# mrcdr/lambda-lanczos

Hardware: AMD Instinct MI355X
Metric: Lanczos iterations/sec + SpMV GB/s (fp64, n=10M nnz=150M) at 1/2/4/8 GPUs (higher is better)
Workload: dtype f64; 1 GPU; random symmetric CSR n=10000000 nnz=150000000 fp64; n=10000000, nnz=150000000, partition=single GPU, orth_mode=0, tridiag_mode=2, eps=engine default

## Files before the change

lambda-lanczos_amd/_capi.py:

```python
import ctypes as C
import os

_HERE = os.path.dirname(os.path.abspath(__file__))
LIB_PATH = os.environ.get("LL_LIB_PATH") or os.path.join(_HERE, "lib", "liblanczos_hip.so")
GEN_PATH = os.path.join(_HERE, "lib", "libllgen.so")
HEADER_PATH = os.path.join(os.path.dirname(_HERE), "include", "lanczos_hip.h")

LL_OK, LL_ERR_INVALID, LL_ERR_HIP, LL_ERR_RCCL, LL_ERR_ALLOC, LL_ERR_CALLBACK = range(6)
ORTH_CGS_DGKS, ORTH_CGS2, ORTH_MGS = 0, 1, 2
TRIDIAG_QR, TRIDIAG_BISECT, TRIDIAG_AUTO = 0, 1, 2
SPMV_CSR_STREAM, SPMV_PB, SPMV_TILED, SPMV_SYM = 0, 1, 2, 3
UPPER, LOWER = 0, 1
ACCURACY_DEFAULT, ACCURACY_NORMWISE, ACCURACY_COMPONENTWISE = 0, 1, 2
UNIQUE_ID_BYTES = 128
EXPO_MULTI_MAX = 16


ABI_VERSION = (0, 5)


class LanczosHipError(RuntimeError):
    def __init__(self, code, msg):
        super().__init__("liblanczos_hip error %d: %s" % (code, msg))
        self.code = code
# ... 65 lines not shown
        ("seconds_host_tridiag", f64),
        ("seconds_spmv", f64),
        ("seconds_orth", f64),
        ("last_alpha_len", i64),
        ("seconds_host_enqueue", f64),
        ("seconds_host_wait", f64),
        ("seconds_setup", f64),
        ("seconds_finish", f64),
        ("second_passes", i64),
        ("seconds_comm_gather", f64),
        ("seconds_comm_allreduce", f64),
        ("lagged_iterations", i64),
        ("pair_iterations", i64),
        ("pair_gate_trips", i64),
        ("workspace_vectors", i64),
        ("replay_mismatches", i64),
        ("reserved", i64 * 4),
    ]

    def as_dict(self):
        d = {k: getattr(self, k) for k, _ in self._fields_ if k != "reserved"}
        d["block_iterations"] = int(self.reserved[0])
        d["block_flushed_vectors"] = int(self.reserved[1])
        return d


P = C.POINTER
PROTOTYPES = {
    "ll_last_error": (C.c_char_p, []),
    "ll_version": (C.c_int, []),
    "ll_abi_check": (C.c_int, [C.c_int, C.c_int, C.c_size_t, C.c_size_t]),
    "ll_ctx_create": (C.c_int, [C.c_int, P(vp)]),
    "ll_ctx_create_on_stream": (C.c_int, [C.c_int, vp, P(vp)]),
    "ll_ctx_destroy": (C.c_int, [vp]),
    "ll_ctx_stream": (C.c_int, [vp, P(vp)]),
    "ll_ctx_synchronize": (C.c_int, [vp]),
    "ll_ctx_release_cache": (C.c_int, [vp]),
    "ll_ctx_reload_env": (C.c_int, [vp]),
    "ll_ctx_set_tuning": (C.c_int, [vp, C.c_char_p, C.c_char_p]),
    "ll_ctx_set_profiling": (C.c_int, [vp, C.c_int]),
    "ll_timer_start": (C.c_int, [vp]),
    "ll_timer_stop": (C.c_int, [vp, P(f64)]),
    "ll_bandwidth_probe": (C.c_int, [vp, C.c_size_t, P(f64), P(f64)]),
    "ll_comm_unique_id": (C.c_int, [vp]),
    "ll_comm_init": (C.c_int, [vp, vp, C.c_int, C.c_int]),
    "ll_comm_rank": (C.c_int, [vp, P(C.c_int), P(C.c_int)]),
# ... 136 lines not shown
```

lambda-lanczos_amd/csrc/context.cpp:

```cpp
#include <algorithm>
#include <cstdlib>
#include <memory>

#include "engine.hpp"

namespace ll {
static thread_local std::string g_last_error;
void set_error(const std::string& msg) { g_last_error = msg; }
}

using namespace ll;

namespace ll {
namespace {
long long to_ll(const std::string& v) { return std::atoll(v.c_str()); }
bool to_flag(const std::string& v) { return std::atoi(v.c_str()) != 0; }
int Tuning::*pauli_bits_key(const std::string& key) {
  static const std::pair<const char*, int Tuning::*> keys[] = {
      {"pauli_tile_bits", &Tuning::pauli_tile_bits}, {"pauli_sector_block_bits", &Tuning::pauli_sector_block_bits},
      {"pauli_momentum_block_bits", &Tuning::pauli_momentum_block_bits},
      {"pauli_momentum_full_block_bits", &Tuning::pauli_momentum_full_block_bits},
      {"pauli_symmetric_block_bits", &Tuning::pauli_symmetric_block_bits},
      {"pauli_block_expand_block_bits", &Tuning::pauli_block_expand_block_bits},
      {"pauli_block_project_block_bits", &Tuning::pauli_block_project_block_bits},
      {"pauli_rdm_tile_bits", &Tuning::pauli_rdm_tile_bits}, {"pauli_rdm_block_bits", &Tuning::pauli_rdm_block_bits}};
  for (const auto& k : keys)
    if (key == k.first) return k.second;
  return nullptr;
}
}
bool tuning_apply(Tuning& t, const std::string& key, const std::string& v) {
  const Tuning d;
  const bool e = v.empty();
  if (key == "spmv_kernel") t.spmv_kernel = v == "csr" ? LL_SPMV_CSR_STREAM : (v == "pb" ? LL_SPMV_PB : (v == "tiled" ? LL_SPMV_TILED : -1));
  else if (key == "spmv_keep_both") t.keep_both = e ? d.keep_both : to_flag(v);
  else if (key == "pb_phase2") t.pb_phase2 = v == "atomic" ? LL_PB_ATOMIC : (v == "ordered" ? LL_PB_ORDERED : LL_PB_FIXED);
  else if (key == "pb_placements") t.pb_placements = e ? d.pb_placements : (int)std::max<long long>(1, std::min<long long>(16, to_ll(v)));
  else if (key == "pb_placement_trace") t.pb_placement_trace = e ? false : to_flag(v);
  else if (key == "comm_overlap") t.comm_overlap = e ? d.comm_overlap : to_flag(v);
  else if (key == "gather_chunks") t.gather_chunks = e ? 0 : (int)std::max<long long>(0, to_ll(v));
  else if (key == "csr_split") t.csr_split = e ? d.csr_split : to_flag(v);
  else if (key == "iter_trace") t.iter_trace = v;
  else if (key == "sharded_norm") t.sharded_norm_measured = v == "measured";
  else if (key == "pair_gs") t.pair_gs = e ? d.pair_gs : to_flag(v);
  else if (key == "block_gs") t.block_gs = e ? d.block_gs : to_flag(v);
  else if (key == "pb_diag") t.pb_diag = e ? d.pb_diag : to_flag(v);
  else if (key == "fuse_launches") {
    const long long level = e ? 2 : to_ll(v);
    t.fuse_launches = level >= 1;
    t.lagged_gs = level >= 2;
  } else if (key == "blas_small_bytes") t.blas_small_bytes = e ? d.blas_small_bytes : to_ll(v);
  else if (key == "tridiag_thread") t.tridiag_thread = e ? d.tridiag_thread : to_flag(v);
  else if (key == "tridiag_lag") t.tridiag_lag = e ? d.tridiag_lag : (int)to_ll(v);
  else if (key == "dgks_threshold") t.dgks_threshold = e ? d.dgks_threshold : std::atof(v.c_str());
  else if (key == "slab_bytes") t.slab_bytes = e ? d.slab_bytes : std::max<long long>(1, to_ll(v));
  else if (key == "pb_block") t.pb_block = e ? 0 : (int)std::max<long long>(0, to_ll(v));
  else if (key == "pb_row_block") t.pb_row_block = e ? 0 : (int)std::max<long long>(0, to_ll(v));
  else if (key == "pb_col_block") t.pb_col_block = e ? 0 : (int)std::max<long long>(0, to_ll(v));
  else if (key == "pb_threads1") {
    t.pb_threads1 = e ? 0 : (int)to_ll(v);
    if (t.pb_threads1 != 256 && t.pb_threads1 != 512 && t.pb_threads1 != 1024) t.pb_threads1 = 0;
  } else if (key == "pb_pad") {
    t.pb_pad = e ? 0 : (int)to_ll(v);
    if (t.pb_pad != 4 && t.pb_pad != 16) t.pb_pad = 0;
  } else if (key == "pb_xpre") t.pb_xpre = e ? d.pb_xpre : to_flag(v);
  else if (key == "pb_test_all_remote") t.pb_test_all_remote = e ? false : to_flag(v);
  else if (key == "force_rp64") t.force_rp64 = e ? false : to_flag(v);
  else if (key == "spmv_tile_balance") t.spmv_tile_balance = e ? d.spmv_tile_balance : to_flag(v);
  else if (int Tuning::*bits = pauli_bits_key(key)) t.*bits = e ? d.*bits : (int)std::max<long long>(0, std::min<long long>(30, to_ll(v)));
// ... 476 lines not shown
```

lambda-lanczos_amd/csrc/engine.hpp:

```cpp
#pragma once

#include <chrono>
#include <complex>
#include <functional>
#include <map>
#include <system_error>
#include <thread>

#include "ll_internal.hpp"

namespace ll {

constexpr int kScalAlpha = 0, kScalNorms = 8, kScalScratch = 32, kScalSpare = 40, kScalZero = 63, kScalCount = 64;

inline double now_s() {
  return std::chrono::duration<double>(std::chrono::steady_clock::now().time_since_epoch()).count();
}
inline int64_t round_up(int64_t v, int64_t m) { return (v + m - 1) / m * m; }
inline bool is_device_ptr(const void* p) {
  if (p == nullptr) return false;
  hipPointerAttribute_t a;
  if (hipPointerGetAttributes(&a, p) != hipSuccess) {
    (void)hipGetLastError();
    return false;
  }
  return a.type == hipMemoryTypeDevice;
}
inline void host_copy(void* dst, const void* src, size_t bytes) {
  constexpr size_t kParallelFrom = (size_t)8 << 20;
  constexpr int kThreads = 4;
  if (bytes < kParallelFrom) {
    std::memcpy(dst, src, bytes);
    return;
  }
  const size_t piece = ((bytes / kThreads) + 4095) & ~(size_t)4095;
  std::thread th[kThreads - 1];
// ... 174 lines not shown
```

lambda-lanczos_amd/csrc/gs_block.hip:

```cpp
#include <algorithm>

#include "gs_strips.hpp"

namespace ll {

namespace {
__device__ __forceinline__ void block_sum2_all(double& a, double& b, double* sh) {
  a = wave_sum(a);
  b = wave_sum(b);
  const int lane = threadIdx.x & 63, wave = threadIdx.x >> 6;
  __syncthreads();
  if (lane == 0) {
    sh[wave] = a;
    sh[4 + wave] = b;
  }
  __syncthreads();
  a = (sh[0] + sh[1]) + (sh[2] + sh[3]);
  b = (sh[4] + sh[5]) + (sh[6] + sh[7]);
}
__device__ __forceinline__ void block_max2_all(double& a, double& b, double* sh) {
#pragma unroll
  for (int d = 32; d > 0; d >>= 1) {
    a = fmax(a, __shfl_down(a, d, 64));
    b = fmax(b, __shfl_down(b, d, 64));
// ... 69 lines not shown
    const double* prev = s == 1 ? dk : p + (size_t)(s - 2) * pstride;
    const double pinv = s == 1 ? 1.0 : 1.0 / sqrt(*sc.nsq[s - 2]);
    const double es = *sc.e[s];
    double* out = p + (size_t)s * pstride;
    for (int i = tid; i < RW; i += 256) {
      const double t = block_tri_row(hist_alpha, hist_beta, in, i, reals, W, alpha_k);
      out[i] = (t - es * in[i]) * inv - nin * (prev[i] * pinv);
    }
    __syncthreads();
  }
  for (int i = tid; i < RW; i += 256) {
    const double ir = 1.0 / sqrt(rho2[i / reals]);
    prA[i] = p[(size_t)(m - 1) * pstride + i] * ir;
    prB[i] = m >= 2 ? p[(size_t)(m - 2) * pstride + i] * ir : 0.0;
  }
}
void launch_block_predict(int k, int m, int reals, const BlockScalars& sc, const double* rho2, const double* cpk, double* hist_alpha,
                          const double* hist_beta, double* dk, double* p, int pstride, double* prA, double* prB, hipStream_t s) {
  hipLaunchKernelGGL(block_predict_kernel, dim3(1), dim3(256), 0, s, k, m, reals, sc, rho2, cpk, hist_alpha, hist_beta, dk, p, pstride, prA,
                     prB);
  LL_HIP(hipGetLastError());
}

template <typename T, int NV, int PC, int M>
__device__ __forceinline__ void block_trip_compute(const T (&ur)[NV][strip<T, PC>::EPT], int nv, const T (&b)[M][strip<T, PC>::EPT],
                                                   T (&cA)[strip<T, PC>::EPT], T (&cB)[strip<T, PC>::EPT],
                                                   const double* __restrict__ prAc, const double* __restrict__ prBc, double* mine,
                                                   int setstride, int lane) {
  constexpr int EPT = strip<T, PC>::EPT;
  double sre[M][NV], sim[M][NV];
#pragma unroll
  for (int v = 0; v < NV; ++v) {
    acc_t<T> ca, cb;
    const int vv = v < nv ? v : nv - 1;
    const bool real = v < nv;
    if constexpr (scalar_traits<T>::is_complex) {
      const double xa = ld_const(prAc, 2 * vv), ya = ld_const(prAc, 2 * vv + 1), xb = ld_const(prBc, 2 * vv), yb = ld_const(prBc, 2 * vv + 1);
      ca = zc{real ? xa : 0.0, real ? ya : 0.0};
      cb = zc{real ? xb : 0.0, real ? yb : 0.0};
    } else {
      const double xa = ld_const(prAc, vv), xb = ld_const(prBc, vv);
      ca = real ? xa : 0.0;
      cb = real ? xb : 0.0;
    }
    acc_t<T> sm[M];
#pragma unroll
    for (int i = 0; i < M; ++i) sm[i] = zero<acc_t<T>>();
#pragma unroll
    for (int e = 0; e < EPT; ++e) {
      fnma_acc(cA[e], ca, ur[v][e]);
      if constexpr (M >= 2) fnma_acc(cB[e], cb, ur[v][e]);
#pragma unroll
// ... 82 lines not shown
      load_lstrip_u<T, PC, FULL>(bv.part[0], base, n, cA);
      if constexpr (M >= 2) load_lstrip_u<T, PC, FULL>(bv.part[1], base, n, cB);
    }
    for (int t = 0; t < ntrips; t += 2) {
      __builtin_amdgcn_sched_barrier(0);
      issue(ub, t + 1);
      __builtin_amdgcn_sched_barrier(0);
      block_trip_compute<T, JB, PC, M>(ua, min(JB, Wl - JB * t), b, cA, cB, prAc + R * JB * t, prBc + R * JB * t, mine + R * JB * t, R * Wl, lane);
      if (t + 1 >= ntrips) break;
      __builtin_amdgcn_sched_barrier(0);
      issue(ua, t + 2);
      __builtin_amdgcn_sched_barrier(0);
      block_trip_compute<T, JB, PC, M>(ub, min(JB, Wl - JB * (t + 1)), b, cA, cB, prAc + R * JB * (t + 1), prBc + R * JB * (t + 1),
                                       mine + R * JB * (t + 1), R * Wl, lane);
    }
    store_lstrip_u<T, PC, FULL>(outA, base, n, cA);
    if constexpr (M >= 2) store_lstrip_u<T, PC, FULL>(outB, base, n, cB);
    if (!last) return;
#pragma unroll
    for (int e = 0; e < EPT; ++e) {
      b[M - 1][e] = cA[e];
      if constexpr (M >= 2) b[M - 2][e] = cB[e];
    }
    int at = 0;
#pragma unroll
    for (int i = 1; i < M; ++i) {
#pragma unroll
      for (int ip = 0; ip < i; ++ip) {
        acc_t<T> g = zero<acc_t<T>>();
#pragma unroll
        for (int e = 0; e < EPT; ++e) cfma_acc(g, b[ip][e], b[i][e]);
        const acc_t<T> gs = wave_sum(g);
        if (lane == 0) {
          if constexpr (scalar_traits<T>::is_complex) {
            tail[at] += gs.re;
            tail[at + 1] += gs.im;
          } else {
            tail[at] += gs;
          }
        }
        at += R;
      }
    }
#pragma unroll
    for (int i = 0; i < M; ++i) {
      double nn = 0.0;
// ... 13 lines not shown
  for (int i = tid; i < lcols; i += kBlock) {
    const double v = (lds[i] + lds[lcols + i]) + (lds[2 * lcols + i] + lds[3 * lcols + i]);
    int g;
    if (i < M * R * Wl) {
      const int set = i / (R * Wl);
      g = set * R * W + R * col0 + (i - set * R * Wl);
    } else {
      g = M * R * W + (i - M * R * Wl);
    }
    out[g] = v;
  }
}
constexpr int kBlockJB = 2;
template <typename T, int PC, int M>
static void block_sweep_launch(int grid, size_t lds_bytes, hipStream_t s, int64_t n, const T* const* vtab, int W, int col0, int Wl, int flags,
                               const BlockVecs<T>& bv, const double* prA, const double* prB, double* partials) {
  hipLaunchKernelGGL((block_sweep_kernel<T, PC, M, kBlockJB>), dim3(grid), dim3(kBlock), lds_bytes, s, n, vtab, W, col0, Wl, flags, bv, prA, prB,
                     partials);
}
template <typename T>
int launch_block_sweep(int64_t n, const T* const* vtab, int W, int m, const BlockVecs<T>& bv, const double* prA, const double* prB,
                       double* partials, int pieces, int per_launch, hipStream_t s) {
  constexpr int R = scalar_traits<T>::reals;
  LL_REQUIRE(m == 1 || m == 2 || m == 4, "internal: block sweep of 1, 2 or 4 iterations");
  const int64_t strips16k = (n * (int64_t)sizeof(T) + 16383) / 16384;
  int pc = strips16k >= kLaggedFullStrips ? 4 : 2;
  if (pieces == 2 || pieces == 4) pc = pieces;
  const int grid = pc == 4 ? strip_grid(n, strip<T, 4>::ELEMS) : strip_grid(n, strip<T, 2>::ELEMS);
  const int ng = R * m * (m - 1) / 2 + m;
  per_launch = std::max(1, std::min(per_launch, block_sweep_max_vecs<T>(m)));
  for (int col0 = 0; col0 < W; col0 += per_launch) {
    const int Wl = std::min(per_launch, W - col0);
    const int flags = (col0 == 0 ? kPairFirst : 0) | (col0 + Wl == W ? kPairLast : 0);
    const size_t lds_bytes = (size_t)4 * (size_t)(m * R * Wl + ((flags & kPairLast) ? ng : 0)) * sizeof(double);
#define LL_BLOCK_SWEEP(PC_, M_) block_sweep_launch<T, PC_, M_>(grid, lds_bytes, s, n, vtab, W, col0, Wl, flags, bv, prA, prB, partials)
    if (pc == 4) {
      if (m == 4) LL_BLOCK_SWEEP(4, 4);
      else if (m == 2) LL_BLOCK_SWEEP(4, 2);
      else LL_BLOCK_SWEEP(4, 1);
    } else {
      if (m == 4) LL_BLOCK_SWEEP(2, 4);
      else if (m == 2) LL_BLOCK_SWEEP(2, 2);
      else LL_BLOCK_SWEEP(2, 1);
    }
#undef LL_BLOCK_SWEEP
    LL_HIP(hipGetLastError());
  }
  return grid;
}

__global__ __launch_bounds__(256) void block_fold_kernel(const double* __restrict__ cols, int k, int m, int reals, BlockScalars sc,
                                                         const double* __restrict__ p, int pstride, double* __restrict__ rho2,
                                                         double* __restrict__ cpk, double* __restrict__ hist_alpha,
                                                         double* __restrict__ hist_beta, double* __restrict__ raw0,
                                                         double* __restrict__ raw1, BlockHost host) {
  __shared__ double red[8];
  const int tid = threadIdx.x;
  const int W = k + 1, RW = reals * W;
  const double* tail = cols + (size_t)m * RW;
  const double* diag = tail + reals * m * (m - 1) / 2;
  for (int s = 0; s < m; ++s) {
    const int j = k + 1 + s;
    double* raw = (s & 1) ? raw1 : raw0;
    const double* rawp = (s & 1) ? raw0 : raw1;
// ... 114 lines not shown
```

lambda-lanczos_amd/csrc/lanczos_loop.hpp:

```cpp
#pragma once

#include "engine.hpp"
#include "loop_support.hpp"
#include "raw_basis.hpp"
#include "ritz_tracker.hpp"
#include "trace.hpp"

#include <algorithm>
#include <cmath>
#include <limits>
#include <random>
#include <string>
#include <variant>

namespace ll {


template <typename T> struct LoopState {
  Engine<T>& E;
  Basis<T>& U;
  EventRing& ring;
  PhaseTimer& timer;
  int64_t nl;
  hipStream_t s;
// ... 44 lines not shown
  int64_t ld = 0;
  int64_t small_bytes = 0;

  int64_t max_k_hint = 0;
  bool pair_enabled = false;
  bool pair_allowed = true;
  int64_t n_pair = 0;
  int64_t n_gate_trips = 0;
  DevBuf<T> pwork[2];
  DevBuf<T> psplit;
  static constexpr size_t kPresizeCols = 4096;
  DevBuf<double> pbuf;
  static constexpr size_t kPairRec = (size_t)kLaggedMaxCols + 32;
  struct PairBuf {
    double* rec[4] = {nullptr, nullptr, nullptr, nullptr};
    double* zero = nullptr;
    double *p3 = nullptr, *p4 = nullptr;
    double* fold = nullptr;
    double* cols = nullptr;
    double* scal = nullptr;
    static constexpr size_t kDoubles = 10 * kPairRec + 64;
  } pb;
  bool slot_pair[kRingSlots] = {};
  int ev_of_slot[kRingSlots] = {0, 1, 2, 3, 4, 5, 6, 7};
  bool block_enabled = false;
  bool block_allowed = true;
  int64_t blk_k0 = 0;
  int64_t n_block = 0;
  int64_t n_block_flushed = 0;
  DevBuf<double> bbuf;
  DevBuf<T> bsplit[2];
  struct BlockBuf {
    double* rho2 = nullptr;
    double* cpk = nullptr;
    double* dk = nullptr;
    double* p = nullptr;
    double *prA = nullptr, *prB = nullptr;
    double *raw0 = nullptr, *raw1 = nullptr;
    double* cols = nullptr;
    double* nsq = nullptr;
    int64_t cap = 0;
    size_t rec = 0;
  } bb;
  static size_t block_row_at(int64_t j) { return ll::block_row_at(Engine<T>::R, j); }
  void enable_block() {
    constexpr size_t R = (size_t)Engine<T>::R;
    block_enabled = true;
    bb.cap = std::min<int64_t>(max_k_hint, (int64_t)kBlockMaxVecs) + 8;
    bb.rec = R * (size_t)(bb.cap + 8);
    const size_t tri = block_row_at(bb.cap) + R * (size_t)bb.cap;
    bbuf.alloc(E.ctx, (size_t)bb.cap + tri + 13 * bb.rec + 64);
    double* b = bbuf.p;
    bb.rho2 = carve(b, (size_t)bb.cap);
    bb.cpk = carve(b, tri);
    bb.dk = carve(b, bb.rec);
    bb.p = carve(b, 4 * bb.rec);
    bb.prA = carve(b, bb.rec);
    bb.prB = carve(b, bb.rec);
    bb.raw0 = carve(b, bb.rec);
    bb.raw1 = carve(b, bb.rec);
    bb.cols = carve(b, 4 * bb.rec + 32);
    bb.nsq = carve(b, 16);
  }
  static constexpr double kGate = sizeof(typename scalar_traits<T>::real) == 4 ? 2e-4 : kPairGate;
  DevBuf<const T*> vtab;
  static constexpr size_t kVtabCap = (size_t)kLaggedMaxCols + (size_t)kLaggedMaxLocked + 64;
  size_t vtab_chunks = 0;
  void vtab_begin_pass() {
    if (!vtab.p) return;
    launch_fill_ptrs<T>(vtab.p, 0, (int)std::min<int64_t>(n_locked, (int64_t)kVtabCap), locked, ld, s);
    vtab_chunks = 0;
  }
  const T* const* vtab_sync() {
    if (!vtab.p) return nullptr;
    for (; vtab_chunks < U.chunks.size(); ++vtab_chunks) {
      const int64_t start = n_locked + (int64_t)vtab_chunks * U.chunk_vecs;
      const int64_t count = std::min<int64_t>(U.chunk_vecs, (int64_t)kVtabCap - start);
      launch_fill_ptrs<T>(vtab.p, (int)start, (int)count, U.chunks[vtab_chunks], ld, s);
    }
    return vtab.p;
  }

  LoopState(Engine<T>& e, Basis<T>& u, EventRing& r, PhaseTimer& t, int64_t n_local, hipStream_t st)
      : E(e), U(u), ring(r), timer(t), nl(n_local), s(st) {}
  void configure(int64_t ld_, int64_t max_iteration, bool orth_dgks, bool defer_ok) {
// ... 45 lines not shown
      size_t p2 = kPresizeCols;
      while (p2 < cols) p2 *= 2;
      cols = p2;
    }
    E.ctx->ensure_partials((size_t)kMaxGrid * cols);
  }
  void bind_buffers() {
    E.ctx->ensure_h(LagBuf::kDoubles);
    double* b = E.ctx->h.get();
    for (auto& g : lb.g) g = carve(b, kHHalf);
    lb.hist_alpha = carve(b, kTOff);
    lb.hist_beta = carve(b, kTOff);
    lb.lambda = carve(b, (size_t)kLaggedMaxLocked);
  }
  void begin_pass(const NormRefs& refs0, const T* locked_vecs, int64_t n_lock, const double* lambda_shifted = nullptr,
                  double offset = 0.0, double norm_scale = 0.0) {
    refs_prev = refs0;
    pending = None{};
    locked = locked_vecs;
    n_locked = n_lock;
    pair_allowed = true;
    block_allowed = true;
    blk_k0 = 0;
    for (auto& b : slot_pair) b = false;
    lag_ok = lagged && n_lock <= kLaggedMaxLocked;
    lag_beta2_min = 0.0;
    if (lag_ok) vtab_begin_pass();
    if (lagged) {
      bind_buffers();
      constexpr size_t R = (size_t)Engine<T>::R;
      const size_t reach = (size_t)std::max<int64_t>(0, std::min<int64_t>(max_k_hint, (int64_t)kLaggedMaxCols)) + (size_t)n_lock + 2;
      const size_t cols = std::min<size_t>(kPresizeCols, (block_enabled ? 4 : 2) * R * reach + 6 * R + 4);
      E.ctx->ensure_partials((size_t)kMaxGrid * cols);
    }
    if (!lag_ok || n_lock == 0) return;
    const bool measure_theta = lambda_shifted == nullptr;
    if (!measure_theta) {
      LL_HIP(hipMemcpyAsync(lb.lambda, lambda_shifted, (size_t)n_lock * sizeof(double), hipMemcpyHostToDevice, s));
      LL_HIP(hipStreamSynchronize(s));
    }
    const BasisSegs<T> none = no_segs<T>(ld);
    E.ctx->ensure_partials(kMaxGrid);
    double* r2_dev = lb.g[0];
    for (int64_t i = 0; i < n_lock; ++i) {
      const T* z = locked + i * ld;
      T* y = work[0].p;
      E.apply(z, y, offset, measure_theta ? lb.lambda + i : nullptr, true);
      const ThreeTerm<T> tt{nullptr, z, lb.lambda + i, NormRefs{nullptr, nullptr, nullptr, 0}};
      const int grid = launch_mdot<T>(nl, y, none, tt, nullptr, E.ctx->partials.get(), small_bytes, s);
      launch_reduce_cols(E.ctx->partials.get(), grid, 1, r2_dev + i, nullptr, s);
    }
    E.all_reduce(r2_dev, (size_t)n_lock);
    std::vector<double> r2((size_t)n_lock), theta;
    E.fetch(r2_dev, r2.data(), (size_t)n_lock);
    if (measure_theta) {
// ... 158 lines not shown
    return basis;
  }
  int64_t enqueue_block(int64_t kk, double offset) {
    if constexpr (sizeof(typename scalar_traits<T>::real) == 8) return enqueue_block_f64(kk, offset);
    else return 0;
  }
  int64_t enqueue_block_f64(int64_t kk, double offset) {
    constexpr int R = Engine<T>::R;
    const Tuning& tune = E.ctx->tune;
    if (!block_enabled || !block_allowed || !pair_allowed || !lag_ok || n_locked != 0) return 0;
    const BlockIter* const bi = pending_as<BlockIter>();
    const LaggedIter* const lg = pending_as<LaggedIter>();
    int64_t k;
    if (bi) {
      if (bi->k + 1 != kk) return 0;
      k = bi->k;
    } else if (lg && lg->k == kk - 1 && kk >= 3) {
      k = kk - 1;
    } else {
      return 0;
    }
    const int64_t remaining = max_k_hint - (kk - 1);
    if (remaining < 1) return 0;
    const int m = remaining >= 4 ? 4 : (remaining >= 2 ? 2 : 1);
    const int64_t strips16k = (nl * (int64_t)sizeof(T) + 16383) / 16384;
    const bool streaming = tune.sweep_pipeline >= 2 || strips16k > 2 * kCUs + kCUs / 4;
    if (!streaming || vec_bytes() < stream_bytes() || k + m + 1 > bb.cap || (size_t)(k + m + 1) > kVtabCap) return 0;
    if (tune.pair_max_stored > 0 && k + 1 > tune.pair_max_stored) return 0;
    const int W = (int)(k + 1);
    const int ncols = m * R * W + R * m * (m - 1) / 2 + m;
    int per_launch = block_sweep_max_vecs<T>(m);
    if (tune.pair_split_vecs > 0) per_launch = std::min(per_launch, std::max(1, tune.pair_split_vecs));
    if (W > per_launch)
      for (auto& b : bsplit)
        if (!b.p) b.alloc(E.ctx, (size_t)ld);
    const double te0 = now_s();
    want_partial_cols((size_t)std::max(ncols, 1 + R));
    if (!bi) {
      LL_HIP(hipMemcpyAsync(U.vec(k), work[k & 1].p, (size_t)nl * sizeof(T), hipMemcpyDeviceToDevice, s));
      launch_block_enter((int)k, R, lb.g[k & 1], lg->c1, bb.rho2, bb.cpk, s);
      blk_k0 = k;
    }
    BlockVecs<T> bv{};
    for (int i = 0; i < m; ++i) bv.b[i] = U.vec(k + 1 + i);
    bv.part[0] = bsplit[0].p;
    bv.part[1] = bsplit[1].p;
    const T* const* vt = vtab_sync();
    BlockScalars sc{};
    BlockHost host{};
    int slots[4] = {0, 0, 0, 0};
    for (int i = 0; i < 4; ++i) {
      const int ii = std::min(i, m - 1);
      slots[i] = (int)((kk + ii) % kRingSlots);
      sc.e[i] = E.S(kScalAlpha + slots[i]);
      sc.nsq[i] = bb.nsq + 4 * ii;
      host.slot[i] = pinned_slot(slots[i]);
      host.gate[i] = pinned_gate(slots[i]);
    }
    for (int i = 0; i < m; ++i) {
      const T* x = i == 0 ? U.vec(k) : bv.b[i - 1];
      const T* xp = i == 0 ? U.vec(k - 1) : (i == 1 ? U.vec(k) : bv.b[i - 2]);
      const double* xn2 = i == 0 ? bb.rho2 + k : bb.nsq + 4 * (i - 1);
      const double* pn2 = i == 0 ? bb.rho2 + k - 1 : (i == 1 ? bb.rho2 + k : bb.nsq + 4 * (i - 2));
      double* e = E.S(kScalAlpha + slots[i]);
      timer.mark();
      typename Engine<T>::DeferredAlpha da;
      E.apply(x, bv.b[i], offset, e, true, fuse_launches ? &da : nullptr, nullptr, xn2);
      timer.mark();
      const int g3 = launch_pair_three_term<T>(nl, bv.b[i], x, xp, e, da.nparts > 0 ? da.partials : nullptr, da.nparts, xn2, pn2,
                                               E.ctx->partials.get(), false, s);
      launch_reduce_cols(E.ctx->partials.get(), g3, 1 + R, bb.nsq + 4 * i, nullptr, s);
      if (i + 1 < m) timer.mark();
    }
    launch_block_predict((int)k, m, R, sc, bb.rho2, bb.cpk, lb.hist_alpha, lb.hist_beta, bb.dk, bb.p, (int)bb.rec, bb.prA, bb.prB, s);
    const int grid = launch_block_sweep<T>(nl, vt, W, m, bv, bb.prA, bb.prB, E.ctx->partials.get(), tune.lagged_pieces, per_launch, s);
    launch_reduce_cols(E.ctx->partials.get(), grid, ncols, bb.cols, nullptr, s);
    const int ev = slots[m - 1];
    launch_block_fold(bb.cols, (int)k, m, R, sc, bb.p, (int)bb.rec, bb.rho2, bb.cpk, lb.hist_alpha, lb.hist_beta, bb.raw0, bb.raw1, host, s,
                      tune.event_in_launch ? ring.ev[ev] : nullptr);
    if (!tune.event_in_launch) LL_HIP(hipEventRecord(ring.ev[ev], s));
    timer.mark();
    for (int i = 0; i < m; ++i) {
      ev_of_slot[slots[i]] = ev;
      slot_pair[slots[i]] = true;
    }
    pending = BlockIter{k + m};
    n_block += m;
    if (m >= 2) n_pair += m;
    n_lagged += m;
    t_enqueue += now_s() - te0;
    return m;
  }
  bool enqueue_pair(int64_t k, double offset) {
    constexpr int R = Engine<T>::R;
    if (!pair_enabled || !pair_allowed || !lag_ok) return false;
    if (max_k_hint > 0 && k + 1 > max_k_hint) return false;
    const int64_t Lk = n_locked;
    PairIter in;
    if (const PairIter* pr = pending_as<PairIter>()) {
      if (pr->P + 2 != k) return false;
      in = *pr;
    } else if (const LaggedIter* lg = pending_as<LaggedIter>(); lg && lg->k == k - 1 && k >= 3) {
      in = PairIter{k - 2, {U.vec(k - 2), work[(k - 1) & 1].p}, {pb.zero, lb.g[(k - 1) & 1]}, {pb.scal + 0, lg->c1}, 0, 1};
    } else {
      return false;
    }
    const int64_t P = in.P;
    const T *const r1 = in.r[0], *const r2 = in.r[1];
    const double *const g1 = in.g[0], *const g2 = in.g[1], *const rho1sq = in.rho2[0], *const rho2sq = in.rho2[1];
    const int out_set = in.set ^ 1, out_rec = in.rec ^ 1;
// ... 200 lines not shown
    }
    RunList<T> runs;
    runs.ld = ld;
    if (full) runs = basis_runs(k);
    enqueue(k, offset, runs, mode);
    return 1;
  }
  void restart_after(int64_t j) {
    pending = None{};
    double* cj = E.S(kScalNorms + 3 * (int)(j % kRingSlots));
    refs_prev = NormRefs{cj, cj + 1, cj + 1, 0};
  }
  struct Scalars {
    double alpha, beta2, c0, c1;
    bool redone;
  };
  Scalars collect(int64_t j) {
    const int slot = (int)(j % kRingSlots);
    const double tw0 = now_s();
    LL_HIP(hipEventSynchronize(ring.ev[ev_of_slot[slot]]));
    t_wait += now_s() - tw0;
    const volatile double* hp = pinned_slot(slot);
    Scalars r{hp[0], hp[1], hp[2], hp[3], false};
    double* const beta2_dev = E.S(kScalNorms + 3 * slot) + 1;
    if (dgks && r.c1 < E.ctx->tune.dgks_threshold * r.c0) {
      if (r.c1 > 0.0 && std::isfinite(r.c1)) {
        const RunList<T> again = basis_runs(j);
        make_final(j);
        r.beta2 = r.c1 * E.second_pass(U.vec(j), again);
        ++n_second_passes;
        launch_set_scalar(beta2_dev, r.beta2, s);
        if (lag_ok) launch_set_scalar(lb.hist_beta + j - 1, std::sqrt(r.beta2), s);
        restart_after(j);
        r.redone = true;
      } else {
        r.beta2 = 0.0;
      }
    }
    if (!r.redone && lag_ok && n_locked > 0 && r.beta2 < lag_beta2_min) {
      make_final(j);
      lag_ok = false;
      restart_after(j);
      r.redone = true;
    }
    if (!r.redone && slot_pair[slot] && !(*pinned_gate(slot) <= kGate)) {
      pair_allowed = false;
// ... 86 lines not shown
  std::mt19937 mt(dev());
  std::uniform_real_distribution<Real> r((Real)-1, (Real)1);
  Real* f = reinterpret_cast<Real*>(v);
  for (int64_t i = 0; i < n * scalar_traits<T>::reals; ++i) f[i] = r(mt);
}

template <typename T>
void fill_stats(ll_run_stats* stats, LoopState<T>& loop, int64_t total_iterations, size_t last_alpha_len, double t_tridiag,
                double t_start) {
  ll_context* ctx = loop.E.ctx;
  if (stats) {
    std::memset(stats, 0, sizeof(*stats));
    stats->total_iterations = total_iterations;
    stats->seconds_host_tridiag = t_tridiag;
    stats->last_alpha_len = (int64_t)last_alpha_len;
    stats->seconds_host_enqueue = loop.t_enqueue;
    stats->seconds_host_wait = loop.t_wait;
    stats->second_passes = loop.n_second_passes;
    stats->lagged_iterations = loop.n_lagged;
    stats->pair_iterations = loop.n_pair;
    stats->pair_gate_trips = loop.n_gate_trips;
    stats->reserved[0] = loop.n_block;
    stats->reserved[1] = loop.n_block_flushed;
    loop.timer.collect(stats->seconds_spmv, stats->seconds_orth);
    ctx->drain_comm_events(&stats->seconds_comm_gather, &stats->seconds_comm_allreduce);
    stats->seconds_total = now_s() - t_start;
  }
  ctx->drain_comm_events(nullptr, nullptr);
}

}
```

lambda-lanczos_amd/csrc/ll_internal.hpp:

```cpp
#pragma once

#include <hip/hip_runtime.h>
#if defined(__HIPCC__)
#include <hip/hip_ext.h>
#endif

#include <algorithm>
#include <atomic>
#include <cstdint>
#include <cstdio>
#include <cstring>
#include <map>
#include <memory>
#include <string>
#include <type_traits>
#include <vector>

#include "../../include/lanczos_hip.h"
#include "../../include/lanczos_hip_transport.h"
#include "scalar_types.hpp"
#include "spmv_plan.hpp"

#if defined(__HIPCC__)
#define LL_LAUNCH_STOP(stop, kernel, grid, block, lds, s, ...)                                      \
// ... 161 lines not shown
  int pb_threads1 = 0;
  int pb_pad = 0;
  int pb_placements = 8;
  bool pb_xpre = true;
  bool pb_diag = true;
  int gather_chunks = 0;
  bool spmv_tile_balance = true;
  bool csr_split = true;
  bool comm_overlap = true;
  bool tridiag_thread = true;
  int tridiag_lag = 3;
  double dgks_threshold = 0.5;
  bool sharded_norm_measured = false;
  int64_t slab_bytes = (int64_t)4 << 30;
  int64_t blas_small_bytes = (int64_t)4 << 20;
  bool fuse_launches = true;
  long long lagged_min_bytes = -1;
  int lagged_pieces = 0;
  bool lagged_gs = true;
  bool event_in_launch = true;
  bool ritz_tail = true;
  int sweep_pipeline = 1;
  bool block_gs = true;
  bool pair_gs = true;
  bool force_rp64 = false;
  bool tl_xcd_order = true;
  bool tl_walk_modulo = true;
  bool tl_force = false;
  bool pb_test_all_remote = false;
  int tridiag_test_jitter_us = 0;
  int pauli_tile_bits = -1;
  int pauli_momentum_block_bits = -1;
  int pauli_momentum_full_block_bits = -1;
  int pauli_symmetric_block_bits = -1;
  int pauli_block_expand_block_bits = -1;
  int pauli_block_project_block_bits = -1;
  int pauli_sector_block_bits = -1;
  int pauli_rdm_tile_bits = -1;
  int pauli_rdm_block_bits = -1;
  int test_workspace_fill = -1;
  bool stencil_vec = true;
  double stall_trace_ms = -1.0;
  std::string iter_trace;
  bool pb_placement_trace = false;
};
Tuning read_tuning(const std::map<std::string, std::string>* overrides);
// ... 431 lines not shown
  const T* u_cur;
  const double* alpha;
  NormRefs prev;
  const double* alpha_partials = nullptr;
  int alpha_nparts = 0;
  double* alpha_out = nullptr;
};
template <typename T>
int launch_mdot(int64_t n, T* w, const BasisSegs<T>& segs, const ThreeTerm<T>& tt, const NormRefs* pred,
                double* partials, int64_t small_bytes, hipStream_t s);
constexpr int kLaggedMaxCols = 5000;
template <typename T> struct Lagged {
  const T* r;
  T* u_out;
  const double* g;
  const double* t;
  const double* beta2;
};
constexpr int kLaggedFullStrips = 200;
template <typename T>
int launch_lagged(int64_t n, T* w, const BasisSegs<T>& segs, const Lagged<T>& lg, const ThreeTerm<T>& tt, double* partials,
                  int pieces, int64_t small_limit, hipStream_t s);
constexpr double kPairGate = 1e-8;
template <typename T>
int launch_pair_three_term(int64_t n, T* y, const T* x, const T* p, double* e, const double* e_partials, int e_nparts,
                           const double* cx2, const double* cp2, double* partials, bool colmajor,
                           hipStream_t s);
void launch_pair_predict(int P, int L, int reals, const double* g1, const double* g2, const double* rho1sq, const double* rho2sq,
                         const double* gam, double* n3sq, const double* d13_partials, int d13_nparts, const double* e1, double* e2,
                         const double* e2_partials, int e2_nparts, const double* hist_alpha, const double* hist_beta,
                         const double* lambda, double* p3, double* p4, hipStream_t s);
constexpr int kPairFirst = 1, kPairLast = 2;
template <typename T> constexpr int pair_sweep_max_vecs() {
  return (kLaggedMaxCols - 5 * scalar_traits<T>::reals - 1) / (2 * scalar_traits<T>::reals);
}
template <typename T>
int launch_pair_sweep(int64_t n, const std::vector<BasisSegs<T>>& groups, int P, const T* r1, const T* r2, const T* r3, T* r4,
                      T* uP_out, T* uQ_out, T* part4, const double* g1, const double* g2, const double* gam, const double* p4,
                      const double* rho1sq, const double* rho2sq, const double* e2, const double* n3sq, double* partials, int pieces,
                      hipStream_t s, const T* const* vtab = nullptr,
                      bool force_pipeline = false);
template <typename T>
bool launch_pair_sweep_small(int64_t n, const BasisSegs<T>& segs, int P, const T* r1, const T* r2, const T* r3, T* r4, T* uP_out,
                             T* uQ_out, const double* g1, const double* g2, const double* gam, const double* p4, const double* rho1sq,
                             const double* rho2sq, const double* e2, const double* n3sq, double* partials, int* grid_out,
                             hipStream_t s);
template <typename T> bool pair_small_fits(int P);
template <typename T> void launch_fill_ptrs(const T** tab, int start, int count, const T* base, int64_t ld, hipStream_t s);
void launch_pair_fold(const double* m, int P, int L, int reals, const double* lambda, const double* p4, const double* g2, const double* gam,
                      const double* rho2sq, const double* n3sq, const double* e1, const double* e2, double* rec3, double* rec4,
                      double* nxt, double* hist_alpha, double* hist_beta, double* scratch, double* host_a, double* host_b,
                      double* gate_a, double* gate_b, hipStream_t s, hipEvent_t stop = nullptr);
constexpr int kBlockMaxVecs = 1024;
struct BlockScalars {
  const double* e[4];
  const double* nsq[4];
};
struct BlockHost {
  double* slot[4];
  double* gate[4];
};
template <typename T> struct BlockVecs {
  T* b[4];
  T* part[2];
};
template <typename T> constexpr int block_sweep_max_vecs(int m) {
  return (kLaggedMaxCols - (scalar_traits<T>::reals * m * (m - 1) / 2 + m)) / (m * scalar_traits<T>::reals);
}
void launch_block_enter(int k, int reals, const double* g, const double* c1, double* rho2, double* cpk, hipStream_t s);
void launch_block_predict(int k, int m, int reals, const BlockScalars& sc, const double* rho2, const double* cpk, double* hist_alpha,
                          const double* hist_beta, double* dk, double* p, int pstride, double* prA, double* prB, hipStream_t s);
template <typename T>
int launch_block_sweep(int64_t n, const T* const* vtab, int W, int m, const BlockVecs<T>& bv, const double* prA, const double* prB,
                       double* partials, int pieces, int per_launch, hipStream_t s);
void launch_block_fold(const double* cols, int k, int m, int reals, const BlockScalars& sc, const double* p, int pstride, double* rho2,
                       double* cpk, double* hist_alpha, double* hist_beta, double* raw0, double* raw1, const BlockHost& host, hipStream_t s,
                       hipEvent_t stop = nullptr);
void launch_lagged_fold(double* m, int K, int L, int reals, double* t_out, const double* c0, double* c0_out, double* c1,
                        double* alpha, const double* prev_g, const double* prev_t, const double* prev_c1,
                        double* hist_alpha, double* hist_beta, const double* lambda, double* host_mapped, hipStream_t s, hipEvent_t stop = nullptr);
template <typename T>
int launch_maxpy(int64_t n, T* w, const BasisSegs<T>& segs, const double* h, const NormRefs* pred, double* partials,
                 int64_t small_bytes, hipStream_t s);
template <typename T>
bool launch_maxpy_folding(int64_t n, T* w, const BasisSegs<T>& segs, const double* mdot_partials, int mparts, double* h_out,
                          double* c0_out, double* partials, int64_t small_bytes, int* grid_out, hipStream_t s);
// ... 57 lines not shown
```

lambda-lanczos_amd/csrc/loop_support.hpp:

```cpp
#pragma once

#include "ll_internal.hpp"

#include <algorithm>
#include <utility>

namespace ll {

template <typename T> struct DevBuf {
  T* p = nullptr;
  ll_context* owner = nullptr;
  size_t bytes = 0;
  ~DevBuf() { release(); }
  void release() {
    if (p && owner) owner->cache_put((void*)p, bytes);
    p = nullptr;
  }
  void alloc(ll_context* ctx, size_t count) {
    release();
    owner = ctx;
    bytes = std::max<size_t>(count * sizeof(T), 16);
    for (size_t i = 0; i < ctx->slab_cache.size(); ++i)
      if (ctx->slab_cache[i].second == bytes) {
        p = (T*)ctx->slab_cache[i].first;
        ctx->slab_cache.erase(ctx->slab_cache.begin() + (long)i);
        break;
      }
    if (!p) ctx->dev_malloc((void**)&p, bytes, "work vectors");
    ctx->test_fill_if_set(p, bytes / sizeof(T));
  }
};

constexpr int kRingSlots = 8, kSlotScalars = 4, kGateAt = kRingSlots * kSlotScalars;
constexpr size_t kPinnedScalars = 48;

struct EventRing {
  hipEvent_t ev[kRingSlots];
  EventRing() {
    for (auto& e : ev) LL_HIP(hipEventCreateWithFlags(&e, hipEventDisableTiming));
  }
  ~EventRing() {
    for (auto& e : ev) (void)hipEventDestroy(e);
  }
};

struct PhaseTimer {
  static constexpr size_t kTriples = 128;
  bool on;
  hipStream_t s;
  std::vector<hipEvent_t>& evs;
  size_t n = 0;
  double acc_op = 0.0, acc_rest = 0.0;
  PhaseTimer(ll_context* ctx, hipStream_t st) : on(ctx->profiling), s(st), evs(ctx->timer_events) {}
  void read(size_t first) {
    float a = 0, b = 0;
    if (hipEventSynchronize(evs[first + 2]) != hipSuccess) return;
    if (hipEventElapsedTime(&a, evs[first], evs[first + 1]) == hipSuccess) acc_op += a * 1e-3;
// ... 35 lines not shown
```

Baseline: 878.8 Lanczos iterations/s.

## Add eight-vector block Gram-Schmidt sweep gated by quiet orthogonality history

```diff
diff --git a/lambda-lanczos_amd/_capi.py b/lambda-lanczos_amd/_capi.py
--- a/lambda-lanczos_amd/_capi.py
+++ b/lambda-lanczos_amd/_capi.py
@@ -111,6 +111,7 @@
         d = {k: getattr(self, k) for k, _ in self._fields_ if k != "reserved"}
         d["block_iterations"] = int(self.reserved[0])
         d["block_flushed_vectors"] = int(self.reserved[1])
+        d["block8_iterations"] = int(self.reserved[2])
         return d
 
 
diff --git a/lambda-lanczos_amd/csrc/context.cpp b/lambda-lanczos_amd/csrc/context.cpp
--- a/lambda-lanczos_amd/csrc/context.cpp
+++ b/lambda-lanczos_amd/csrc/context.cpp
@@ -44,7 +44,11 @@
   else if (key == "sharded_norm") t.sharded_norm_measured = v == "measured";
   else if (key == "pair_gs") t.pair_gs = e ? d.pair_gs : to_flag(v);
   else if (key == "block_gs") t.block_gs = e ? d.block_gs : to_flag(v);
-  else if (key == "pb_diag") t.pb_diag = e ? d.pb_diag : to_flag(v);
+  else if (key == "block_gs_max") {
+    const long long m = e ? d.block_gs_max : to_ll(v);
+    if (m != 4 && m != 8) return false;
+    t.block_gs_max = (int)m;
+  } else if (key == "pb_diag") t.pb_diag = e ? d.pb_diag : to_flag(v);
   else if (key == "fuse_launches") {
     const long long level = e ? 2 : to_ll(v);
     t.fuse_launches = level >= 1;
diff --git a/lambda-lanczos_amd/csrc/engine.hpp b/lambda-lanczos_amd/csrc/engine.hpp
--- a/lambda-lanczos_amd/csrc/engine.hpp
+++ b/lambda-lanczos_amd/csrc/engine.hpp
@@ -11,7 +11,7 @@
 
 namespace ll {
 
-constexpr int kScalAlpha = 0, kScalNorms = 8, kScalScratch = 32, kScalSpare = 40, kScalZero = 63, kScalCount = 64;
+constexpr int kScalAlpha = 0, kScalNorms = 16, kScalScratch = 64, kScalSpare = 72, kScalZero = 127, kScalCount = 128;
 
 inline double now_s() {
   return std::chrono::duration<double>(std::chrono::steady_clock::now().time_since_epoch()).count();
diff --git a/lambda-lanczos_amd/csrc/gs_block.hip b/lambda-lanczos_amd/csrc/gs_block.hip
--- a/lambda-lanczos_amd/csrc/gs_block.hip
+++ b/lambda-lanczos_amd/csrc/gs_block.hip
@@ -115,12 +115,85 @@
   LL_HIP(hipGetLastError());
 }
 
+template <int CTRL> __device__ __forceinline__ double dpp_move(double v) {
+  const int lo = __builtin_amdgcn_update_dpp(0, __double2loint(v), CTRL, 0xf, 0xf, false);
+  const int hi = __builtin_amdgcn_update_dpp(0, __double2hiint(v), CTRL, 0xf, 0xf, false);
+  return __hiloint2double(hi, lo);
+}
+__device__ __forceinline__ void swap_add32(double& x, double y) {
+  const auto lo = __builtin_amdgcn_permlane32_swap((unsigned)__double2loint(x), (unsigned)__double2loint(y), false, false);
+  const auto hi = __builtin_amdgcn_permlane32_swap((unsigned)__double2hiint(x), (unsigned)__double2hiint(y), false, false);
+  x = __hiloint2double((int)hi[0], (int)lo[0]) + __hiloint2double((int)hi[1], (int)lo[1]);
+}
+__device__ __forceinline__ void swap_add16(double& x, double y) {
+  const auto lo = __builtin_amdgcn_permlane16_swap((unsigned)__double2loint(x), (unsigned)__double2loint(y), false, false);
+  const auto hi = __builtin_amdgcn_permlane16_swap((unsigned)__double2hiint(x), (unsigned)__double2hiint(y), false, false);
+  x = __hiloint2double((int)hi[0], (int)lo[0]) + __hiloint2double((int)hi[1], (int)lo[1]);
+}
+__device__ __forceinline__ void wave_sum_transposed8(double (&a)[8], int lane) {
+#pragma unroll
+  for (int i = 0; i < 4; ++i) swap_add32(a[i], a[i + 4]);
+#pragma unroll
+  for (int i = 0; i < 2; ++i) swap_add16(a[i], a[i + 2]);
+  const bool upper = (lane & 8) != 0;
+  const double keep = upper ? a[1] : a[0], send = upper ? a[0] : a[1];
+  double v = keep + dpp_move<0x128>(send);
+  v += dpp_move<0x141>(v);
+  v += dpp_move<0x4e>(v);
+  v += dpp_move<0xb1>(v);
+  a[0] = v;
+}
+
+template <typename T, int NV, int PC>
+__device__ __forceinline__ void block_trip_compute8(const T (&ur)[NV][strip<T, PC>::EPT], int nv, const T (&b)[8][strip<T, PC>::EPT],
+                                                    T (&cA)[strip<T, PC>::EPT], T (&cB)[strip<T, PC>::EPT],
+                                                    const double* __restrict__ prAc, const double* __restrict__ prBc, double* mine,
+                                                    int setstride, int lane) {
+  constexpr int EPT = strip<T, PC>::EPT;
+  constexpr int H = 4, NF = H * NV, LPF = 64 / NF;
+  static_assert(!scalar_traits<T>::is_complex && NF == 8, "the sweep of eight: real double, two stored vectors per trip");
+#pragma unroll
+  for (int v = 0; v < NV; ++v) {
+    const int vv = v < nv ? v : nv - 1;
+    const bool real = v < nv;
+    const double xa = ld_const(prAc, vv), xb = ld_const(prBc, vv);
+    const double ca = real ? xa : 0.0, cb = real ? xb : 0.0;
+#pragma unroll
+    for (int e = 0; e < EPT; ++e) {
+      fnma_acc(cA[e], ca, ur[v][e]);
+      fnma_acc(cB[e], cb, ur[v][e]);
+    }
+  }
+  const int f = lane / LPF, fv = f / H, fi = f % H;
+#pragma unroll
+  for (int h = 0; h < 8 / H; ++h) {
+    double fs[NF];
+#pragma unroll
+    for (int v = 0; v < NV; ++v) {
+#pragma unroll
+      for (int i = 0; i < H; ++i) {
+        double sm = 0.0;
+#pragma unroll
+        for (int e = 0; e < EPT; ++e) cfma_acc(sm, ur[v][e], b[h * H + i][e]);
+        fs[v * H + i] = sm;
+      }
+    }
+    wave_sum_transposed8(fs, lane);
+    if ((lane & (LPF - 1)) == 0 && fv < nv) mine[(h * H + fi) * setstride + fv] += fs[0];
+    __builtin_amdgcn_sched_barrier(0);
+  }
+}
+
 template <typename T, int NV, int PC, int M>
 __device__ __forceinline__ void block_trip_compute(const T (&ur)[NV][strip<T, PC>::EPT], int nv, const T (&b)[M][strip<T, PC>::EPT],
                                                    T (&cA)[strip<T, PC>::EPT], T (&cB)[strip<T, PC>::EPT],
                                                    const double* __restrict__ prAc, const double* __restrict__ prBc, double* mine,
                                                    int setstride, int lane) {
   constexpr int EPT = strip<T, PC>::EPT;
+  if constexpr (M == 8) {
+    block_trip_compute8<T, NV, PC>(ur, nv, b, cA, cB, prAc, prBc, mine, setstride, lane);
+    return;
+  }
   double sre[M][NV], sim[M][NV];
 #pragma unroll
   for (int v = 0; v < NV; ++v) {
@@ -249,6 +322,55 @@
       b[M - 1][e] = cA[e];
       if constexpr (M >= 2) b[M - 2][e] = cB[e];
     }
+    if constexpr (M == 8) {
+      constexpr int NP = M * (M - 1) / 2;
+      static_assert(NP + 4 == 32 && !scalar_traits<T>::is_complex, "the Gram triangle of eight and four norms fill two reductions of 16");
+      const int f = lane >> 2;
+      auto half = [&](auto first_c) {
+        constexpr int FIRST = decltype(first_c)::value;
+        double ga[16];
+        int a = 0;
+#pragma unroll
+        for (int i = 1; i < M; ++i) {
+#pragma unroll
+          for (int ip = 0; ip < i; ++ip) {
+            if (a >= FIRST && a < FIRST + 16) {
+              double g = 0.0;
+#pragma unroll
+              for (int e = 0; e < EPT; ++e) cfma_acc(g, b[ip][e], b[i][e]);
+              ga[a - FIRST] = g;
+            }
+            ++a;
+          }
+        }
+        if constexpr (FIRST == 16) {
+#pragma unroll
+          for (int i = 0; i < 4; ++i) {
+            double n0 = 0.0;
+#pragma unroll
+            for (int e = 0; e < EPT; ++e) n0 += abs2(b[i][e]);
+            ga[NP - 16 + i] = n0;
+          }
+        }
+        wave_sum_transposed<16>(ga, lane);
+        if ((lane & 3) == 0) tail[FIRST + f] += ga[0];
+        if constexpr (FIRST == 16) {
+#pragma unroll
+          for (int i = 4; i < M; ++i) {
+            double nn = 0.0;
+#pragma unroll
+            for (int e = 0; e < EPT; ++e) nn += abs2(b[i][e]);
+            nn = wave_sum(nn);
+            if (lane == 0) tail[NP + i] += nn;
+          }
+        }
+      };
+      __builtin_amdgcn_sched_barrier(0);
+      half(std::integral_constant<int, 0>{});
+      __builtin_amdgcn_sched_barrier(0);
+      half(std::integral_constant<int, 16>{});
+      return;
+    }
     int at = 0;
 #pragma unroll
     for (int i = 1; i < M; ++i) {
@@ -308,10 +430,11 @@
 int launch_block_sweep(int64_t n, const T* const* vtab, int W, int m, const BlockVecs<T>& bv, const double* prA, const double* prB,
                        double* partials, int pieces, int per_launch, hipStream_t s) {
   constexpr int R = scalar_traits<T>::reals;
-  LL_REQUIRE(m == 1 || m == 2 || m == 4, "internal: block sweep of 1, 2 or 4 iterations");
+  LL_REQUIRE(m == 1 || m == 2 || m == 4 || m == 8, "internal: block sweep of 1, 2, 4 or 8 iterations");
   const int64_t strips16k = (n * (int64_t)sizeof(T) + 16383) / 16384;
   int pc = strips16k >= kLaggedFullStrips ? 4 : 2;
   if (pieces == 2 || pieces == 4) pc = pieces;
+  if (m == 8) pc = 2;
   const int grid = pc == 4 ? strip_grid(n, strip<T, 4>::ELEMS) : strip_grid(n, strip<T, 2>::ELEMS);
   const int ng = R * m * (m - 1) / 2 + m;
   per_launch = std::max(1, std::min(per_launch, block_sweep_max_vecs<T>(m)));
@@ -325,7 +448,10 @@
       else if (m == 2) LL_BLOCK_SWEEP(4, 2);
       else LL_BLOCK_SWEEP(4, 1);
     } else {
-      if (m == 4) LL_BLOCK_SWEEP(2, 4);
+      if (m == 8) {
+        if constexpr (scalar_traits<T>::is_complex) LL_REQUIRE(false, "internal: the block sweep of eight is built for real double only");
+        else LL_BLOCK_SWEEP(2, 8);
+      } else if (m == 4) LL_BLOCK_SWEEP(2, 4);
       else if (m == 2) LL_BLOCK_SWEEP(2, 2);
       else LL_BLOCK_SWEEP(2, 1);
     }
diff --git a/lambda-lanczos_amd/csrc/lanczos_loop.hpp b/lambda-lanczos_amd/csrc/lanczos_loop.hpp
--- a/lambda-lanczos_amd/csrc/lanczos_loop.hpp
+++ b/lambda-lanczos_amd/csrc/lanczos_loop.hpp
@@ -90,12 +90,16 @@
     static constexpr size_t kDoubles = 10 * kPairRec + 64;
   } pb;
   bool slot_pair[kRingSlots] = {};
-  int ev_of_slot[kRingSlots] = {0, 1, 2, 3, 4, 5, 6, 7};
+  static_assert(kRingSlots == 16 && kScalNorms >= kScalAlpha + kRingSlots && kScalScratch >= kScalNorms + 3 * kRingSlots,
+                "the rings of the device scalar area follow kRingSlots");
+  int ev_of_slot[kRingSlots] = {0, 1, 2, 3, 4, 5, 6, 7, 8, 9, 10, 11, 12, 13, 14, 15};
   bool block_enabled = false;
   bool block_allowed = true;
   int64_t blk_k0 = 0;
   int64_t n_block = 0;
   int64_t n_block_flushed = 0;
+  int64_t n_block8 = 0;
+  int blk_quiet = 0;
   DevBuf<double> bbuf;
   DevBuf<T> bsplit[2];
   struct BlockBuf {
@@ -117,18 +121,19 @@
     bb.cap = std::min<int64_t>(max_k_hint, (int64_t)kBlockMaxVecs) + 8;
     bb.rec = R * (size_t)(bb.cap + 8);
     const size_t tri = block_row_at(bb.cap) + R * (size_t)bb.cap;
-    bbuf.alloc(E.ctx, (size_t)bb.cap + tri + 13 * bb.rec + 64);
+    constexpr size_t kTail = R * (size_t)(kBlockMaxM * (kBlockMaxM - 1) / 2) + (size_t)kBlockMaxM;
+    bbuf.alloc(E.ctx, (size_t)bb.cap + tri + (5 + 2 * (size_t)kBlockMaxM) * bb.rec + kTail + 4 * (size_t)kBlockMaxM + 32);
     double* b = bbuf.p;
     bb.rho2 = carve(b, (size_t)bb.cap);
     bb.cpk = carve(b, tri);
     bb.dk = carve(b, bb.rec);
-    bb.p = carve(b, 4 * bb.rec);
+    bb.p = carve(b, (size_t)kBlockMaxM * bb.rec);
     bb.prA = carve(b, bb.rec);
     bb.prB = carve(b, bb.rec);
     bb.raw0 = carve(b, bb.rec);
     bb.raw1 = carve(b, bb.rec);
-    bb.cols = carve(b, 4 * bb.rec + 32);
-    bb.nsq = carve(b, 16);
+    bb.cols = carve(b, (size_t)kBlockMaxM * bb.rec + kTail);
+    bb.nsq = carve(b, 4 * (size_t)kBlockMaxM);
   }
   static constexpr double kGate = sizeof(typename scalar_traits<T>::real) == 4 ? 2e-4 : kPairGate;
   DevBuf<const T*> vtab;
@@ -220,6 +225,7 @@
     pair_allowed = true;
     block_allowed = true;
     blk_k0 = 0;
+    blk_quiet = 0;
     for (auto& b : slot_pair) b = false;
     lag_ok = lagged && n_lock <= kLaggedMaxLocked;
     lag_beta2_min = 0.0;
@@ -228,7 +234,7 @@
       bind_buffers();
       constexpr size_t R = (size_t)Engine<T>::R;
       const size_t reach = (size_t)std::max<int64_t>(0, std::min<int64_t>(max_k_hint, (int64_t)kLaggedMaxCols)) + (size_t)n_lock + 2;
-      const size_t cols = std::min<size_t>(kPresizeCols, (block_enabled ? 4 : 2) * R * reach + 6 * R + 4);
+      const size_t cols = std::min<size_t>(kPresizeCols, (block_enabled ? (size_t)E.ctx->tune.block_gs_max : 2) * R * reach + 6 * R + 4);
       E.ctx->ensure_partials((size_t)kMaxGrid * cols);
     }
     if (!lag_ok || n_lock == 0) return;
@@ -433,7 +439,8 @@
     }
     const int64_t remaining = max_k_hint - (kk - 1);
     if (remaining < 1) return 0;
-    const int m = remaining >= 4 ? 4 : (remaining >= 2 ? 2 : 1);
+    const bool eight = !scalar_traits<T>::is_complex && tune.block_gs_max >= 8 && remaining >= 8 && blk_quiet >= kBlock8Quiet;
+    const int m = eight ? 8 : (remaining >= 4 ? 4 : (remaining >= 2 ? 2 : 1));
     const int64_t strips16k = (nl * (int64_t)sizeof(T) + 16383) / 16384;
     const bool streaming = tune.sweep_pipeline >= 2 || strips16k > 2 * kCUs + kCUs / 4;
     if (!streaming || vec_bytes() < stream_bytes() || k + m + 1 > bb.cap || (size_t)(k + m + 1) > kVtabCap) return 0;
@@ -459,8 +466,8 @@
     const T* const* vt = vtab_sync();
     BlockScalars sc{};
     BlockHost host{};
-    int slots[4] = {0, 0, 0, 0};
-    for (int i = 0; i < 4; ++i) {
+    int slots[kBlockMaxM] = {};
+    for (int i = 0; i < kBlockMaxM; ++i) {
       const int ii = std::min(i, m - 1);
       slots[i] = (int)((kk + ii) % kRingSlots);
       sc.e[i] = E.S(kScalAlpha + slots[i]);
@@ -497,6 +504,7 @@
     }
     pending = BlockIter{k + m};
     n_block += m;
+    if (m == 8) n_block8 += m;
     if (m >= 2) n_pair += m;
     n_lagged += m;
     t_enqueue += now_s() - te0;
@@ -743,6 +751,7 @@
     t_wait += now_s() - tw0;
     const volatile double* hp = pinned_slot(slot);
     Scalars r{hp[0], hp[1], hp[2], hp[3], false};
+    blk_quiet = block_enabled && slot_pair[slot] && *pinned_gate(slot) <= kBlock8Tau ? std::min(blk_quiet + 1, (int)kBlock8Quiet) : 0;
     double* const beta2_dev = E.S(kScalNorms + 3 * slot) + 1;
     if (dgks && r.c1 < E.ctx->tune.dgks_threshold * r.c0) {
       if (r.c1 > 0.0 && std::isfinite(r.c1)) {
@@ -875,6 +884,7 @@
     stats->pair_gate_trips = loop.n_gate_trips;
     stats->reserved[0] = loop.n_block;
     stats->reserved[1] = loop.n_block_flushed;
+    stats->reserved[2] = loop.n_block8;
     loop.timer.collect(stats->seconds_spmv, stats->seconds_orth);
     ctx->drain_comm_events(&stats->seconds_comm_gather, &stats->seconds_comm_allreduce);
     stats->seconds_total = now_s() - t_start;
diff --git a/lambda-lanczos_amd/csrc/ll_internal.hpp b/lambda-lanczos_amd/csrc/ll_internal.hpp
--- a/lambda-lanczos_amd/csrc/ll_internal.hpp
+++ b/lambda-lanczos_amd/csrc/ll_internal.hpp
@@ -207,6 +207,7 @@
   bool ritz_tail = true;
   int sweep_pipeline = 1;
   bool block_gs = true;
+  int block_gs_max = 8;
   bool pair_gs = true;
   bool force_rp64 = false;
   bool tl_xcd_order = true;
@@ -684,6 +685,8 @@
 int launch_lagged(int64_t n, T* w, const BasisSegs<T>& segs, const Lagged<T>& lg, const ThreeTerm<T>& tt, double* partials,
                   int pieces, int64_t small_limit, hipStream_t s);
 constexpr double kPairGate = 1e-8;
+constexpr double kBlock8Tau = 5e-14;
+constexpr int kBlock8Quiet = 12;
 template <typename T>
 int launch_pair_three_term(int64_t n, T* y, const T* x, const T* p, double* e, const double* e_partials, int e_nparts,
                            const double* cx2, const double* cp2, double* partials, bool colmajor,
@@ -714,16 +717,17 @@
                       double* nxt, double* hist_alpha, double* hist_beta, double* scratch, double* host_a, double* host_b,
                       double* gate_a, double* gate_b, hipStream_t s, hipEvent_t stop = nullptr);
 constexpr int kBlockMaxVecs = 1024;
+constexpr int kBlockMaxM = 8;
 struct BlockScalars {
-  const double* e[4];
-  const double* nsq[4];
+  const double* e[kBlockMaxM];
+  const double* nsq[kBlockMaxM];
 };
 struct BlockHost {
-  double* slot[4];
-  double* gate[4];
+  double* slot[kBlockMaxM];
+  double* gate[kBlockMaxM];
 };
 template <typename T> struct BlockVecs {
-  T* b[4];
+  T* b[kBlockMaxM];
   T* part[2];
 };
 template <typename T> constexpr int block_sweep_max_vecs(int m) {
diff --git a/lambda-lanczos_amd/csrc/loop_support.hpp b/lambda-lanczos_amd/csrc/loop_support.hpp
--- a/lambda-lanczos_amd/csrc/loop_support.hpp
+++ b/lambda-lanczos_amd/csrc/loop_support.hpp
@@ -31,8 +31,8 @@
   }
 };
 
-constexpr int kRingSlots = 8, kSlotScalars = 4, kGateAt = kRingSlots * kSlotScalars;
-constexpr size_t kPinnedScalars = 48;
+constexpr int kRingSlots = 16, kSlotScalars = 4, kGateAt = kRingSlots * kSlotScalars;
+constexpr size_t kPinnedScalars = 96;
 
 struct EventRing {
   hipEvent_t ev[kRingSlots];
```

Result: faster. 945.4 Lanczos iterations/s, median of 6 (+7.6%).
